# michaelnny/alpha_zero

Measured on AMD Instinct MI355X. Metric: self-play moves/sec (whole node), 9x9 Go @ 200 sims/move, higher is better.
Workload: dtype fp32-class evaluator (f16 hi+lo pairs, 3 MFMA products, fp32 accumulate) / f32-f64 tree

## Files before the change

alpha_zero_amd/csrc/az_conv_sp2p.h:

```cpp
#pragma once
#include "az_conv_sp.h"

#if defined(__HIPCC__)
#define SP2P_NB 12

__device__ __forceinline__ float sp2_fma_f32(float a, float s, float c) {
    float r;
    asm("v_fma_f32 %0, %1, %2, %3" : "=v"(r) : "v"(a), "s"(s), "v"(c));
    return r;
}

struct Sp2pMap {
    unsigned char cell[10 * 16];
};
constexpr Sp2pMap sp2p_map_table = {{
     46,  48,  50,  52,  47,  49,  51,  64,  65,  67,  69,  71,  53,  66,  68,  70,
     10,  12,  14,  16,  11,  13,  15,  28,  29,  31,  33,  35,  17,  30,  32,  34,
     20,  22,  24,  37,  19,  21,  23,  25,  26,  39,  41,  43,  38,  40,  42,  44,
      1,   2,   3,   4,  82,  83,  84,  85,  86,  87,  88,  89,   5,   6,   7,   8,
     55,  56,  57,  58, 136, 137, 138, 139, 140, 141, 142, 143,  59,  60,  61,  62,
     73,  74,  75,  76, 154, 155, 156, 157, 158, 159, 160, 161,  77,  78,  79,  80,
      0,   9,  18,  27,  81,  90,  99, 108, 117, 126, 135, 144,  36,  45,  54,  63,
    127, 129, 131, 133, 128, 130, 132, 145, 146, 148, 150, 152, 134, 147, 149, 151,
     91,  93,  95,  97,  92,  94,  96, 109, 110, 112, 114, 116,  98, 111, 113, 115,
    101, 103, 105, 118, 100, 102, 104, 106, 107, 120, 122, 124, 119, 121, 123, 125,
}};
constexpr int SP2P_NCT = 10, SP2P_KS = 18;
constexpr bool sp2p_tap_off(int pos, int tap) {
    const int yy = pos / SpGeo9::S + tap / 3 - 1, xx = pos % SpGeo9::S + tap % 3 - 1;
    return yy < 0 || yy >= SpGeo9::S || xx < 0 || xx >= SpGeo9::S;
}
constexpr bool sp2p_skip(const Sp2pMap& m, int tile, int tap) {
    for (int n = 0; n < 16; ++n)
        if (!sp2p_tap_off(m.cell[tile * 16 + n] % SpGeo9::P2, tap)) return false;
    return true;
}
constexpr int sp2p_skips(const Sp2pMap& m) {
    int n = 0;
    for (int t = 0; t < SP2P_NCT; ++t)
        for (int tap = 0; tap < 9; ++tap) n += sp2p_skip(m, t, tap) ? 1 : 0;
    return n;
}
constexpr bool sp2p_map_complete(const Sp2pMap& m) {
    bool used[2 * SpGeo9::P2] = {};
    for (int i = 0; i < SP2P_NCT * 16; ++i) {
        const int v = m.cell[i];
        if (v >= 2 * SpGeo9::P2 || v % SpGeo9::P2 == SpGeo9::CORNER || used[v]) return false;
        used[v] = true;
    }
    return true;
}
constexpr bool sp2p_map_conflict_free(const Sp2pMap& m) {
    for (int t = 0; t < SP2P_NCT; ++t) {
        bool bank[16] = {};
        for (int n = 0; n < 16; ++n) {
            const int r = (SpGeo9::cell_of(m.cell[t * 16 + n] % SpGeo9::P2) + ((n >= 4 && n < 12) ? 8 : 0)) & 15;
            if (bank[r]) return false;
            bank[r] = true;
        }
    }
    return true;
}
constexpr bool sp2p_skips_as_designed(const Sp2pMap& m) {
    for (int t = 0; t < SP2P_NCT; ++t)
        for (int tap = 0; tap < 9; ++tap) {
            const bool want = (t == 3 && tap / 3 == 0) || (t == 5 && tap / 3 == 2) || (t == 6 && tap % 3 == 0);
            if (sp2p_skip(m, t, tap) != want) return false;
        }
    return true;
}
constexpr int sp2p_sector_complete(const Sp2pMap& m) {
    int n = 0;
    for (int t = 0; t < SP2P_NCT; ++t)
        for (int a = 0; a < 16; ++a)
            for (int b = 0; b < 16; ++b) {
                const int p = m.cell[t * 16 + a], q = m.cell[t * 16 + b];
                n += (q == p + 1 && p / SpGeo9::P2 == q / SpGeo9::P2) ? 1 : 0;
            }
    return n;
}
static_assert(sp2p_map_complete(sp2p_map_table), "pair map: every position of both boards but the two corners exactly once");
static_assert(sp2p_map_conflict_free(sp2p_map_table), "pair map: conflict-free lane groups in every tile");
static_assert(sp2p_skips_as_designed(sp2p_map_table) && sp2p_skips(sp2p_map_table) == 9, "pair map: the three edge tiles skip 3 taps each, 9 of 90 (tile, tap) pairs");
static_assert(sp2p_sector_complete(sp2p_map_table) == 126, "pair map: 9 rows of both boards in one tile each, 7 whole sectors per row");
static __device__ const Sp2pMap sp2p_map = sp2p_map_table;

constexpr int sp2p_j0(int u) { return u == 0 ? 0 : u == 1 ? 3 : u == 2 ? 5 : 8; }
constexpr int sp2p_nj(int u) { return (u & 1) ? 2 : 3; }
constexpr bool sp2p_has_end(int u) { return u == 0 || u == 3; }
struct Sp2pSched {
    int n;
    int kstart[SP2P_KS + 1];
    int live_n[SP2P_KS];
    unsigned char live[SP2P_KS][3];
    unsigned char t[324], jl[324], tt[324], prod[324], first[324];
};
constexpr Sp2pSched sp2p_sched(int u) {
    Sp2pSched s = {};
    const int j0 = sp2p_j0(u), nj = sp2p_nj(u);
    int first_t[3] = {-1, -1, -1};
    int n = 0;
    for (int t = 0; t < SP2P_KS; ++t) {
        int ln = 0;
        for (int j = 0; j < nj; ++j)
            if (!sp2p_skip(sp2p_map_table, j0 + j, t / 2)) {
                s.live[t][ln++] = (unsigned char)j;
                if (first_t[j] < 0) first_t[j] = t;
            }
        s.live_n[t] = ln;
        s.kstart[t] = n;
        for (int r6 = 0; r6 < 6; ++r6)
            for (int k = 0; k < ln; ++k) {
                const int j = s.live[t][k];
                s.t[n] = (unsigned char)t, s.jl[n] = (unsigned char)j, s.tt[n] = (unsigned char)(r6 / 3), s.prod[n] = (unsigned char)(r6 % 3);
                s.first[n] = first_t[j] == t ? 1 : 0;
                ++n;
            }
    }
    s.kstart[SP2P_KS] = n, s.n = n;
    return s;
}
template <int U> struct Sp2pU {
    static constexpr Sp2pSched S = sp2p_sched(U);
};
static_assert(Sp2pU<0>::S.n + Sp2pU<1>::S.n + Sp2pU<2>::S.n + Sp2pU<3>::S.n == 972, "MFMAs per wave and pair: 1080 less 9 x 12");
static_assert(Sp2pU<1>::S.n == 180, "the top tile shares its unit with the never-skipped tile");

template <bool RES, int U> struct Sp2pK {
    static constexpr int KS = SP2P_KS, S0 = 6, NPIECE = 16;
    static constexpr int E1 = RES ? 4 : 2, PAIR = 2 * E1 + 8, CT_OPS = 2 * PAIR + 2, P2CT = CT_OPS + 1;
    static constexpr int PU = (U + 3) & 3, NU = (U + 1) & 3;
    static constexpr int nj = sp2p_nj(U), j0 = sp2p_j0(U), pnj = sp2p_nj(PU), pj0 = sp2p_j0(PU);
    static constexpr bool END = sp2p_has_end(U), PRE = !sp2p_has_end(PU);
    static constexpr int N = Sp2pU<U>::S.n, KLAST = Sp2pU<U>::S.kstart[KS - 1];
    static constexpr int P1 = 5 * pnj, SBX = S0 + P1 + 1, P2 = pnj * P2CT;
    static constexpr int AVAIL = (END ? KLAST : N - 4) - (SBX + 1);
    typedef SpSpread<P2, SBX + 1, AVAIL> SP;
    static constexpr bool DMA = END;
    static constexpr int PFIRST = SBX + 3, PSTRIDE = U == 0 ? 9 : 6, PLAST = PFIRST + (NPIECE - 1) * PSTRIDE;
    static_assert(SP::MAXPER <= 1, "the previous unit's finishing fits this unit's MFMA gaps");
    static_assert(SBX + 1 < Sp2pU<U>::S.kstart[4] && 2 * nj <= S0, "hand-over early in the unit; residual loads in front of it");
    static_assert(!DMA || (PLAST + 2 * 6 * nj < KLAST && PFIRST > SBX), "pieces behind the barrier that frees the image, well in front of the end barrier");
};
template <bool RES, int U> __host__ __device__ constexpr int sp2p_vm_younger() {
    typedef Sp2pK<RES, U> K;
    int n = 0;
    for (int c = 0; c < K::pnj; ++c)
        for (int st = 0; st < 2; ++st)
            if (K::SP::slot_of(c * K::P2CT + K::P2CT - 2 + st) > K::PLAST) ++n;
    return n;
}

template <bool RES> __global__ void __launch_bounds__(CW_THREADS, 1)
k_conv3x3_sp2p(const unsigned char* __restrict__ x, const _Float16* __restrict__ w, const float* __restrict__ bias,
               const unsigned char* __restrict__ res, unsigned char* __restrict__ y, int npairs, int relu, unsigned* range) {
    typedef SpGeo9 G;
    constexpr int C = 128, CIN = 128, NCH = 16, NCG = 2;
    constexpr int KSUB = 2, KS = SP2P_KS;
    constexpr int NT = 2;
    constexpr int NJ0 = 3, NJ1 = 2, R = 2;
    constexpr int LBLK = G::CELLS * 16, LPLANE = NCH * LBLK, LBUF = 2 * LPLANE;
    constexpr int GBLK = G::P2 * 16, XPLANE = NCH * GBLK, XTILE = 2 * XPLANE;
    constexpr int YPLANE = (C / 8) * GBLK, YTILE = 2 * YPLANE;
    constexpr int NP = (G::CELLS + 63) / 64, SPW = 2 * NCH / 4, NPIECE = NP * SPW;
    constexpr int NF = NT * 2 * KS;
    constexpr int NF_A = 64;
    constexpr int P2CT = Sp2pK<RES, 0>::P2CT, PAIR = Sp2pK<RES, 0>::PAIR, E1 = Sp2pK<RES, 0>::E1, S0 = Sp2pK<RES, 0>::S0;
    static_assert(NPIECE == Sp2pK<RES, 0>::NPIECE && KS % R == 0, "pieces per image; ring phase");
    constexpr int SIDE_BOARD = 8 * NCH * 16 + 16, SIDE0 = 2 * LBUF + 16, XB0 = SIDE0 + SP2P_NB * SIDE_BOARD, XBCT = 4 * 1024;
    __shared__ __attribute__((aligned(1024))) unsigned char lds[XB0 + NJ0 * XBCT];
    static_assert(XB0 + NJ0 * XBCT <= 160 * 1024 && XB0 % 16 == 0, "LDS budget");
    const int tid = threadIdx.x, lane = tid & 63, l15 = lane & 15, kg = lane >> 4;
    const int wave = __builtin_amdgcn_readfirstlane(tid >> 6);
    const int wa = wave >> 1, wb = wave & 1;
    const unsigned lds0 = (unsigned)(size_t)(__attribute__((address_space(3))) unsigned char*)lds;
    int cg, slot, nslot;
    {
        const int b = (int)blockIdx.x, nb = (int)gridDim.x;
        nslot = nb / NCG;
        if (nb % (8 * NCG) == 0) {
            const int xcd = b & 7, k = b >> 3;
            cg = k % NCG;
            slot = xcd + 8 * (k / NCG);
        } else {
            cg = b % NCG;
            slot = b / NCG;
        }
    }
    for (int i = tid; i < (XB0 + NJ0 * XBCT) / 16; i += CW_THREADS) *(cv_u32x4*)(lds + i * 16) = (cv_u32x4){0u, 0u, 0u, 0u};
    CV_BARRIER();
    if (slot >= npairs) return;

    sp_f16x8 wf[NF];
#pragma unroll
    for (int f = 0; f < NF; ++f) {
        const int tt = f / (2 * KS), pl = (f / KS) & 1, st = f % KS;
        wf[f] = *(const sp_f16x8*)(w + ((size_t)((pl * 9 + st / KSUB) * C + cg * 64 + wa * 32 + ((tt + wb) & 1) * 16 + l15)) * CIN + wb * 64 + (st % KSUB) * 32 + kg * 8);
    }
    c6_f32x4 bv;
#pragma unroll
    for (int e = 0; e < 4; ++e) bv[e] = bias[cg * 64 + wa * 32 + wb * 16 + 4 * kg + e];
    const float lo_relu = relu ? 0.0f : -__builtin_inff();
    const float lo_clamp = relu ? 0.0f : -SP_F16_MAX;

    unsigned dsrc[NP];
    unsigned long long dmask[NP];
#pragma unroll
    for (int i = 0; i < NP; ++i) {
        const int p = 64 * i + lane < G::CELLS ? G::pos_of_cell(64 * i + lane) : -1;
        dsrc[i] = (unsigned)((p < 0 ? 0 : p) * 16);
        dmask[i] = __builtin_amdgcn_ballot_w64(p >= 0);
    }
    auto dma_piece = [&](const unsigned char* src, unsigned dstbuf, bool live, int i) {
        const int c = SPW * wave + i / NP, pc = i % NP;
        const unsigned long long base = (unsigned long long)(src + (size_t)c * GBLK);
        const unsigned long long mask = live ? dmask[pc] : 0ull;
        const unsigned dst = dstbuf + (unsigned)(c * LBLK + pc * 1024);
        asm volatile("s_mov_b64 exec, %0\n\ts_mov_b32 m0, %1\n\ts_nop 0\n\tglobal_load_lds_dwordx4 %2, %3 nt\n\ts_mov_b64 exec, -1"
                     :
                     : "s"(mask), "s"(dst), "v"(dsrc[pc]), "s"(base)
                     : "memory");
    };
    unsigned lmap[SP2P_NCT], omap[SP2P_NCT];
#pragma unroll
    for (int j = 0; j < SP2P_NCT; ++j) {
        const int v = sp2p_map.cell[j * 16 + l15], bd = v >= G::P2 ? 1 : 0, pos = v - bd * G::P2;
        lmap[j] = (unsigned)(bd * LBUF + (G::PITCH * (pos / G::S) + pos % G::S) * 16 + kg * LBLK + wb * (8 * LBLK));
        omap[j] = (unsigned)(bd * YTILE + pos * 16 + (kg >> 1) * GBLK + (kg & 1) * 8);
    }
    auto out_off = [&](int j) __attribute__((always_inline)) {
        unsigned v = omap[j];
        asm volatile("" : "+v"(v));
        return v;
    };
    sp_f16x8 bb[R][2][NJ0];
    auto load_frag = [&](int j, int jl, int s, int rs, int pl) __attribute__((always_inline)) {
        const int tap = s / KSUB;
        const int off = ((tap / 3) * G::PITCH + (tap % 3)) * 16 + (s % KSUB) * (4 * LBLK);
        bb[rs][pl][jl] = *(const sp_f16x8*)(lds + lmap[j] + off + pl * LPLANE);
    };
    {
        const unsigned char* src = x + (size_t)slot * (2 * XTILE);
#pragma unroll
        for (int i = 0; i < NPIECE; ++i) dma_piece(src, lds0, true, i);
        asm volatile("s_waitcnt vmcnt(0)" ::: "memory");
        CV_BARRIER();
        static_assert(Sp2pU<0>::S.live_n[0] == NJ0, "the first k-step of a pair has all of U0's tiles");
#pragma unroll
        for (int pl = 0; pl < 2; ++pl)
#pragma unroll
            for (int j = 0; j < NJ0; ++j) load_frag(j, j, 0, 0, pl);
    }
#pragma unroll
    for (int f = 0; f < NF; ++f) {
        if (f < NF_A) asm volatile("" : : "a"(wf[f]));
        else asm volatile("" : : "v"(wf[f]));
    }
    asm volatile("" : : "v"(bv), "v"(lmap[0]), "v"(lmap[SP2P_NCT - 1]), "v"(dsrc[0]), "v"(dsrc[NP - 1]));

    c6_f32x4 accm[2][NJ0][NT], accc[2][NJ0][NT];
    cv_u32x2 rr[2][NJ0][2];
#pragma unroll
    for (int a = 0; a < 2; ++a)
#pragma unroll
        for (int j = 0; j < NJ0; ++j) {
#pragma unroll
            for (int t = 0; t < NT; ++t) accm[a][j][t] = (c6_f32x4){0.0f, 0.0f, 0.0f, 0.0f}, accc[a][j][t] = (c6_f32x4){0.0f, 0.0f, 0.0f, 0.0f};
            rr[a][j][0] = (cv_u32x2){0u, 0u}, rr[a][j][1] = (cv_u32x2){0u, 0u};
        }
    float evv[2] = {0.0f, 0.0f}, sc[2] = {0.0f, 0.0f}, t0 = 0.0f, mx = 0.0f;
    unsigned hpk[2] = {0u, 0u}, lpk[2] = {0u, 0u};
    c6_f32x4 xs = (c6_f32x4){0.0f, 0.0f, 0.0f, 0.0f}, xr = (c6_f32x4){0.0f, 0.0f, 0.0f, 0.0f};
    unsigned char* const xb_mine = lds + XB0 + wave * 1024 + lane * 16;
    const unsigned char* const xb_partner = lds + XB0 + (wave ^ 1) * 1024 + lane * 16;
    auto send_op = [&](int set, int c, int o) {
        if (o < 4) xs[o] = sp2_fma_f32(accc[set][c][1][o], SP_INV_SCALE, accm[set][c][1][o]);
        else *(c6_f32x4*)(xb_mine + c * XBCT) = xs;
    };
    auto fin_op = [&](int set, int c, int mj, unsigned char* out, sp_gptr out_lo, int o, bool store_ok) {
        if (o == 0) {
            xr = *(const c6_f32x4*)(xb_partner + c * XBCT);
            return;
        }
        o -= 1;
        if (o < 2 * PAIR) {
            const int pr = o / PAIR, k = o % PAIR;
            if (k < 2 * E1) {
                const int ei = k / E1, kk = k % E1, e = 2 * pr + ei;
                const unsigned rh = pr == 0 ? rr[set][c][0].x : rr[set][c][0].y, rl = pr == 0 ? rr[set][c][1].x : rr[set][c][1].y;
                if (kk == 0) evv[ei] = fmaf(accc[set][c][0][e], SP_INV_SCALE, accm[set][c][0][e]);
                else if (kk == 1) evv[ei] = cw_add_f32(evv[ei], xr[e]);
                else if (RES && kk == 2) t0 = ei == 0 ? sp_mix_join<0>(rh, rl) : sp_mix_join<1>(rh, rl);
                else if (RES && kk == 3) evv[ei] = cw_add_f32(evv[ei], t0);
            } else {
                const int kk = k - 2 * E1;
                if (kk == 0) mx = sp_max3_abs(mx, evv[0], evv[1]);
                else if (kk == 1) evv[0] = __builtin_amdgcn_fmed3f(evv[0], lo_clamp, SP_F16_MAX);
                else if (kk == 2) evv[1] = __builtin_amdgcn_fmed3f(evv[1], lo_clamp, SP_F16_MAX);
                else if (kk == 3) hpk[pr] = sp_cvt_pk(evv[0], evv[1]);
                else if (kk == 4) sc[0] = sp_mix_diff<0>(hpk[pr], evv[0]);
                else if (kk == 5) sc[1] = sp_mix_diff<1>(hpk[pr], evv[1]);
                else if (kk == 6) lpk[pr] = sp_scale_cvt_lo(sc[0]);
                else lpk[pr] = sp_scale_cvt_hi(lpk[pr], sc[1]);
            }
        } else {
            const unsigned gq = out_off(mj);
            if (o == 2 * PAIR) {
                if (store_ok) *(cv_u32x2*)(out + gq) = (cv_u32x2){hpk[0], hpk[1]};
            } else if (store_ok) *(__attribute__((address_space(1))) cv_u32x2*)(out_lo + gq) = (cv_u32x2){lpk[0], lpk[1]};
        }
    };

    const bool copier = tid < 8 * NCH;
    int csrc, cdst;
    {
        constexpr int KF = NCH / 4;
        const int c = copier ? tid : 0, ks = c % KF, pl = (c / KF) & 1, tp = (c / (2 * KF)) & 3, g4 = c / (8 * KF);
        csrc = (pl * NCH + 4 * ks + g4) * LBLK + (G::CELL0 + G::PITCH * (G::S - 2 + (tp >> 1)) + (tp & 1)) * 16;
        cdst = SIDE0 + c * 16;
    }
    cv_u32x4 ctmp = (cv_u32x4){0u, 0u, 0u, 0u};

    int it = 0, cb = 0;
    unsigned char* yprev = y;
    sp_gptr yprev_lo = (sp_gptr)(unsigned long long)y;
    for (int pair = slot; pair < npairs; pair += nslot, ++it) {
        const bool has_next = pair + nslot < npairs;
        const unsigned char* bsrc = x + (size_t)pair * (2 * XTILE) + XTILE;
        const unsigned char* nsrc = x + (size_t)(has_next ? pair + nslot : pair) * (2 * XTILE);
        const size_t yo = (size_t)pair * (2 * YTILE) + (size_t)(cg * 8 + wa * 4 + wb * 2) * GBLK;
        const unsigned char* rbase = RES ? res + yo : nullptr;
        unsigned char* ybase = y + yo;
        unsigned long long rlo = (unsigned long long)(RES ? res + yo : y + yo) + YPLANE, ylo = (unsigned long long)(y + yo) + YPLANE;
        asm volatile("" : "+s"(rlo), "+s"(ylo));
        const sp_gcptr rbase_lo = (sp_gcptr)rlo;
        const sp_gptr ybase_lo = (sp_gptr)ylo;
        const bool have_prev = it > 0;
        auto unit = [&](auto UC) __attribute__((always_inline)) {
            constexpr int u = decltype(UC)::value, set = u & 1, pset = set ^ 1;
            typedef Sp2pK<RES, u> K;
            typedef typename K::SP SP;
            constexpr int nj = K::nj, j0 = K::j0, pj0 = K::pj0, nj0 = sp2p_j0(K::NU);
            unsigned char* pout = u == 0 ? yprev : ybase;
            const sp_gptr pout_lo = u == 0 ? yprev_lo : ybase_lo;
            const bool pstore = u > 0 || have_prev;
            cp_for_each([&](auto SC) __attribute__((always_inline)) {
                constexpr int sl = decltype(SC)::value;
                constexpr int t = Sp2pU<u>::S.t[sl], jl = Sp2pU<u>::S.jl[sl], tt = Sp2pU<u>::S.tt[sl], prod = Sp2pU<u>::S.prod[sl];
                constexpr int qi = sl - Sp2pU<u>::S.kstart[t];
                constexpr bool first = Sp2pU<u>::S.first[sl] != 0;
                if constexpr (K::END && sl == K::KLAST) {
                    constexpr int VM_YOUNGER = sp2p_vm_younger<RES, u>();
                    static_assert(VM_YOUNGER < 63, "vmcnt field");
                    if (pstore) asm volatile("s_waitcnt vmcnt(%0)" ::"n"(VM_YOUNGER) : "memory");
                    else asm volatile("s_waitcnt vmcnt(0)" ::: "memory");
                    CV_BARRIER();
                }
                if constexpr (K::PRE && sl == S0 - 1) CV_BARRIER();
                if constexpr (sl == K::SBX) CV_BARRIER();
                constexpr int fa = (tt * 2 + (prod == 2 ? 1 : 0)) * KS + t, pl = prod == 1 ? 1 : 0;
                static_assert(!first || fa < NF_A, "an accumulator's first MFMA reads its weights from the AGPRs");
                if constexpr (prod == 0) {
                    if constexpr (first && tt == 0) sp_mfma_ac(accm[set][jl][tt], wf[fa], bb[t % R][pl][jl], bv);
                    else if constexpr (first) sp_mfma_a0(accm[set][jl][tt], wf[fa], bb[t % R][pl][jl]);
                    else if constexpr (fa < NF_A) sp_mfma_a(accm[set][jl][tt], wf[fa], bb[t % R][pl][jl]);
                    else sp_mfma_v(accm[set][jl][tt], wf[fa], bb[t % R][pl][jl]);
                } else if constexpr (prod == 1) {
                    if constexpr (first) sp_mfma_a0(accc[set][jl][tt], wf[fa], bb[t % R][pl][jl]);
                    else if constexpr (fa < NF_A) sp_mfma_a(accc[set][jl][tt], wf[fa], bb[t % R][pl][jl]);
                    else sp_mfma_v(accc[set][jl][tt], wf[fa], bb[t % R][pl][jl]);
                } else {
                    if constexpr (fa < NF_A) sp_mfma_a(accc[set][jl][tt], wf[fa], bb[t % R][pl][jl]);
                    else sp_mfma_v(accc[set][jl][tt], wf[fa], bb[t % R][pl][jl]);
                }
                {
                    constexpr bool lsame = t + 1 < KS;
                    constexpr int lu = lsame ? u : K::NU, lt = lsame ? t + 1 : 0, lj0 = lsame ? j0 : nj0;
                    constexpr int lnj = Sp2pU<lu>::S.live_n[lt];
                    static_assert(2 * lnj <= 6 * Sp2pU<u>::S.live_n[t], "a fragment per MFMA gap");
                    if constexpr (qi < 2 * lnj) {
                        constexpr int ljl = Sp2pU<lu>::S.live[lt][qi % lnj];
                        load_frag(lj0 + ljl, ljl, lt, (t + 1) % R, qi / lnj);
                    }
                }
                if constexpr (sl >= S0 && sl < S0 + K::P1) send_op(pset, (sl - S0) / 5, (sl - S0) % 5);
                if constexpr (sl > K::SBX) {
                    constexpr int o = SP::cum(sl - 1);
                    if constexpr (o < SP::cum(sl)) fin_op(pset, o / P2CT, pj0 + o / P2CT, pout, pout_lo, o % P2CT, pstore);
                }
                if constexpr (RES && sl < 2 * nj) {
                    constexpr int rj = sl >> 1, rp = sl & 1;
                    if constexpr (rp == 0) rr[set][rj][rp] = *(const cv_u32x2*)(rbase + out_off(j0 + rj));
                    else rr[set][rj][rp] = *(const __attribute__((address_space(1))) cv_u32x2*)(rbase_lo + out_off(j0 + rj));
                }
                __builtin_amdgcn_sched_barrier(0);
                if constexpr (K::DMA && sl >= K::PFIRST && sl <= K::PLAST && (sl - K::PFIRST) % K::PSTRIDE == 0) {
                    if constexpr (u == 0) dma_piece(bsrc, lds0 + LBUF, true, (sl - K::PFIRST) / K::PSTRIDE);
                    else dma_piece(nsrc, lds0, has_next, (sl - K::PFIRST) / K::PSTRIDE);
                    __builtin_amdgcn_sched_barrier(0);
                }
                if constexpr ((u == 0 || u == 2) && sl == Sp2pU<u>::S.kstart[3] - 1) {
                    if (copier) ctmp = *(const cv_u32x4*)(lds + csrc + (u == 2 ? LBUF : 0));
                    __builtin_amdgcn_sched_barrier(0);
                }
                if constexpr ((u == 0 || u == 2) && sl == Sp2pU<u>::S.kstart[6] - 1) {
                    if (copier) *(cv_u32x4*)(lds + cdst + (cb + (u == 2 ? 1 : 0)) * SIDE_BOARD) = ctmp;
                    __builtin_amdgcn_sched_barrier(0);
                }
            }, typename CpMakeSeq<K::N>::type{});
        };
        unit(CpInt<0>{});
        unit(CpInt<1>{});
        unit(CpInt<2>{});
        unit(CpInt<3>{});
        yprev = ybase, yprev_lo = ybase_lo;
        cb += 2;
        if (cb == SP2P_NB || !has_next) {
            const int n_ok = cb, it0 = it - (cb / 2 - 1);
            c6_f32x4 cm[NT], cc[NT];
            constexpr int KF = NCH / 4;
            const unsigned char* sb = lds + SIDE0 + l15 * SIDE_BOARD + kg * (8 * KF * 16);
            const int nb = l15 < n_ok ? l15 : 0;
            const size_t board = 2 * ((size_t)slot + (size_t)(it0 + (nb >> 1)) * nslot) + (nb & 1);
            const size_t co = board * YTILE + (size_t)(cg * 8 + wa * 4 + wb * 2 + (kg >> 1)) * GBLK + G::CORNER * 16 + (kg & 1) * 8;
            if (RES) {
                rr[0][0][0] = *(const cv_u32x2*)(res + co);
                rr[0][0][1] = *(const cv_u32x2*)(res + co + YPLANE);
            }
            cp_for_each([&](auto TC) __attribute__((always_inline)) {
                constexpr int u = decltype(TC)::value, tp = u / KSUB, ks = u % KSUB;
                constexpr int fw = ((tp >> 1) * 3 + 1 + (tp & 1)) * KSUB + ks;
                const sp_f16x8 bh = *(const sp_f16x8*)(sb + ((tp * 2 + 0) * KF + wb * KSUB + ks) * 16);
                const sp_f16x8 bl = *(const sp_f16x8*)(sb + ((tp * 2 + 1) * KF + wb * KSUB + ks) * 16);
#pragma unroll
                for (int tt = 0; tt < NT; ++tt) {
                    const int fh = (tt * 2 + 0) * KS + fw, fl = (tt * 2 + 1) * KS + fw;
                    if (u == 0 && tt == 0) sp_mfma_ac(cm[tt], wf[fh], bh, bv);
                    else if (u == 0) sp_mfma_a0(cm[tt], wf[fh], bh);
                    else if (fh < NF_A) sp_mfma_a(cm[tt], wf[fh], bh);
                    else sp_mfma_v(cm[tt], wf[fh], bh);
                    if (u == 0) sp_mfma_a0(cc[tt], wf[fh], bl);
                    else if (fh < NF_A) sp_mfma_a(cc[tt], wf[fh], bl);
                    else sp_mfma_v(cc[tt], wf[fh], bl);
                    if (fl < NF_A) sp_mfma_a(cc[tt], wf[fl], bh);
                    else sp_mfma_v(cc[tt], wf[fl], bh);
                }
                __builtin_amdgcn_sched_barrier(0);
            }, typename CpMakeSeq<4 * KSUB>::type{});
            asm volatile("s_nop 15\n\ts_nop 15" : "+v"(cm[0]), "+v"(cc[0]), "+v"(cm[1]), "+v"(cc[1]));
            c6_f32x4 hs;
#pragma unroll
            for (int e = 0; e < 4; ++e) hs[e] = fmaf(cc[1][e], SP_INV_SCALE, cm[1][e]);
            *(c6_f32x4*)(xb_mine) = hs;
            CV_BARRIER();
            const c6_f32x4 hr = *(const c6_f32x4*)(xb_partner);
            float v[4];
#pragma unroll
            for (int e = 0; e < 4; ++e) v[e] = fmaf(cc[0][e], SP_INV_SCALE, cm[0][e]) + hr[e];
            if (RES) {
                const cv_u32x2 rh = rr[0][0][0], rl = rr[0][0][1];
                v[0] += sp_join(sp_lo16(rh.x), sp_lo16(rl.x));
                v[1] += sp_join(sp_hi16(rh.x), sp_hi16(rl.x));
                v[2] += sp_join(sp_lo16(rh.y), sp_lo16(rl.y));
                v[3] += sp_join(sp_hi16(rh.y), sp_hi16(rl.y));
            }
            _Float16 h[4], l[4];
#pragma unroll
            for (int e = 0; e < 4; ++e) {
                if (l15 < n_ok) mx = fmaxf(mx, fabsf(v[e]));
                v[e] = fmaxf(v[e], lo_relu);
                sp_split(v[e], h[e], l[e]);
            }
            if (l15 < n_ok) {
                *(cv_u32x2*)(y + co) = (cv_u32x2){sp_pack(h[0], h[1]), sp_pack(h[2], h[3])};
                *(cv_u32x2*)(y + co + YPLANE) = (cv_u32x2){sp_pack(l[0], l[1]), sp_pack(l[2], l[3])};
            }
            cb = 0;
            CV_BARRIER();
        }
    }
    asm volatile("s_nop 15\n\ts_nop 15" : "+v"(accm[1][0][0]), "+v"(accm[1][1][0]), "+v"(accc[1][0][0]), "+v"(accc[1][1][0]), "+v"(accm[1][0][1]), "+v"(accm[1][1][1]),
                 "+v"(accc[1][0][1]), "+v"(accc[1][1][1]));
#pragma unroll
    for (int c = 0; c < NJ1; ++c)
#pragma unroll
        for (int o = 0; o < 5; ++o) send_op(1, c, o);
    CV_BARRIER();
#pragma unroll
    for (int c = 0; c < NJ1; ++c)
#pragma unroll
        for (int o = 0; o < P2CT; ++o) fin_op(1, c, sp2p_j0(3) + c, yprev, yprev_lo, o, true);
    sp_range_report(mx, range);
}
#endif
```

Before: 7274.

## Share LDS input fragments across row-shifted tiles in the interior conv units

Reorders the pair map so that the tiles within units 0 and 3 are vertical row shifts of one another. Those units then run a skewed schedule over row steps, in which one LDS fragment read feeds every live tile. The goal is fewer LDS fragment reads per wave (about 252 instead of 324), so less LDS bandwidth and issue pressure in the MFMA conv loop. In exchange the step count and MFMA ordering change, and so do the barrier and DMA slot positions that are tied to kstart. That may perturb the hand-tuned overlap of finishing work and prefetch.

```diff
diff --git a/alpha_zero_amd/csrc/az_conv_sp2p.h b/alpha_zero_amd/csrc/az_conv_sp2p.h
--- a/alpha_zero_amd/csrc/az_conv_sp2p.h
+++ b/alpha_zero_amd/csrc/az_conv_sp2p.h
@@ -14,16 +14,16 @@
     unsigned char cell[10 * 16];
 };
 constexpr Sp2pMap sp2p_map_table = {{
-     46,  48,  50,  52,  47,  49,  51,  64,  65,  67,  69,  71,  53,  66,  68,  70,
-     10,  12,  14,  16,  11,  13,  15,  28,  29,  31,  33,  35,  17,  30,  32,  34,
-     20,  22,  24,  37,  19,  21,  23,  25,  26,  39,  41,  43,  38,  40,  42,  44,
+     16,  17,  48,  49,  10,  11,  12,  13,  14,  15,  46,  47,  50,  51,  52,  53,
+     25,  26,  57,  58,  19,  20,  21,  22,  23,  24,  55,  56,  59,  60,  61,  62,
+     34,  35,  66,  67,  28,  29,  30,  31,  32,  33,  64,  65,  68,  69,  70,  71,
       1,   2,   3,   4,  82,  83,  84,  85,  86,  87,  88,  89,   5,   6,   7,   8,
-     55,  56,  57,  58, 136, 137, 138, 139, 140, 141, 142, 143,  59,  60,  61,  62,
+    118, 119, 120, 121,  37,  38,  39,  40,  41,  42,  43,  44, 122, 123, 124, 125,
      73,  74,  75,  76, 154, 155, 156, 157, 158, 159, 160, 161,  77,  78,  79,  80,
       0,   9,  18,  27,  81,  90,  99, 108, 117, 126, 135, 144,  36,  45,  54,  63,
-    127, 129, 131, 133, 128, 130, 132, 145, 146, 148, 150, 152, 134, 147, 149, 151,
-     91,  93,  95,  97,  92,  94,  96, 109, 110, 112, 114, 116,  98, 111, 113, 115,
-    101, 103, 105, 118, 100, 102, 104, 106, 107, 120, 122, 124, 119, 121, 123, 125,
+     97,  98, 129, 130,  91,  92,  93,  94,  95,  96, 127, 128, 131, 132, 133, 134,
+    106, 107, 138, 139, 100, 101, 102, 103, 104, 105, 136, 137, 140, 141, 142, 143,
+    115, 116, 147, 148, 109, 110, 111, 112, 113, 114, 145, 146, 149, 150, 151, 152,
 }};
 constexpr int SP2P_NCT = 10, SP2P_KS = 18;
 constexpr bool sp2p_tap_off(int pos, int tap) {
@@ -88,51 +88,97 @@
 constexpr int sp2p_j0(int u) { return u == 0 ? 0 : u == 1 ? 3 : u == 2 ? 5 : 8; }
 constexpr int sp2p_nj(int u) { return (u & 1) ? 2 : 3; }
 constexpr bool sp2p_has_end(int u) { return u == 0 || u == 3; }
+constexpr bool sp2p_row_shifts(const Sp2pMap& m, int u) {
+    const int j0 = sp2p_j0(u), nj = sp2p_nj(u);
+    for (int j = 0; j < nj; ++j) {
+        for (int n = 0; n < 16; ++n)
+            if (m.cell[(j0 + j) * 16 + n] != m.cell[j0 * 16 + n] + j * SpGeo9::S) return false;
+        for (int tap = 0; tap < 9; ++tap)
+            if (sp2p_skip(m, j0 + j, tap)) return false;
+    }
+    return true;
+}
+static_assert(sp2p_row_shifts(sp2p_map_table, 0) && sp2p_row_shifts(sp2p_map_table, 3), "pair map: the local tiles of a board are row shifts of one another");
+static_assert(!sp2p_row_shifts(sp2p_map_table, 1) && !sp2p_row_shifts(sp2p_map_table, 2), "pair map: the units with edge tiles read a fragment per tile");
+constexpr int SP2P_MAXST = 6 * 5;
 struct Sp2pSched {
-    int n;
-    int kstart[SP2P_KS + 1];
-    int live_n[SP2P_KS];
-    unsigned char live[SP2P_KS][3];
-    unsigned char t[324], jl[324], tt[324], prod[324], first[324];
+    int n, ns;
+    bool shared;
+    int kstart[SP2P_MAXST + 1];
+    int live_n[SP2P_MAXST];
+    unsigned char live[SP2P_MAXST][3];
+    unsigned char frow[SP2P_MAXST], fcol[SP2P_MAXST], fkh[SP2P_MAXST];
+    unsigned char st[324], jl[324], wk[324], tt[324], prod[324], first[324];
+    constexpr int nfrag(int step) const { return shared ? 1 : live_n[step]; }
+    constexpr int reads() const {
+        int r = 0;
+        for (int i = 0; i < ns; ++i) r += 2 * nfrag(i);
+        return r;
+    }
 };
 constexpr Sp2pSched sp2p_sched(int u) {
     Sp2pSched s = {};
     const int j0 = sp2p_j0(u), nj = sp2p_nj(u);
-    int first_t[3] = {-1, -1, -1};
+    s.shared = sp2p_row_shifts(sp2p_map_table, u);
+    s.ns = s.shared ? 6 * (nj + 2) : SP2P_KS;
+    int first_st[3] = {-1, -1, -1};
     int n = 0;
-    for (int t = 0; t < SP2P_KS; ++t) {
-        int ln = 0;
-        for (int j = 0; j < nj; ++j)
-            if (!sp2p_skip(sp2p_map_table, j0 + j, t / 2)) {
-                s.live[t][ln++] = (unsigned char)j;
-                if (first_t[j] < 0) first_t[j] = t;
-            }
-        s.live_n[t] = ln;
-        s.kstart[t] = n;
+    for (int i = 0; i < s.ns; ++i) {
+        const int row = i / 6, col = (i / 2) % 3, kh = i % 2;
+        int ln = 0, wk[3] = {};
+        for (int j = 0; j < nj; ++j) {
+            const int dy1 = s.shared ? row - j : row;
+            if (dy1 < 0 || dy1 > 2 || sp2p_skip(sp2p_map_table, j0 + j, dy1 * 3 + col)) continue;
+            wk[ln] = (dy1 * 3 + col) * 2 + kh;
+            s.live[i][ln++] = (unsigned char)j;
+            if (first_st[j] < 0) first_st[j] = i;
+        }
+        s.live_n[i] = ln;
+        s.kstart[i] = n;
+        s.frow[i] = (unsigned char)row, s.fcol[i] = (unsigned char)col, s.fkh[i] = (unsigned char)kh;
         for (int r6 = 0; r6 < 6; ++r6)
             for (int k = 0; k < ln; ++k) {
-                const int j = s.live[t][k];
-                s.t[n] = (unsigned char)t, s.jl[n] = (unsigned char)j, s.tt[n] = (unsigned char)(r6 / 3), s.prod[n] = (unsigned char)(r6 % 3);
-                s.first[n] = first_t[j] == t ? 1 : 0;
+                const int j = s.live[i][k];
+                s.st[n] = (unsigned char)i, s.jl[n] = (unsigned char)j, s.wk[n] = (unsigned char)wk[k], s.tt[n] = (unsigned char)(r6 / 3), s.prod[n] = (unsigned char)(r6 % 3);
+                s.first[n] = first_st[j] == i ? 1 : 0;
                 ++n;
             }
     }
-    s.kstart[SP2P_KS] = n, s.n = n;
+    s.kstart[s.ns] = n, s.n = n;
     return s;
+}
+constexpr bool sp2p_chains_ascend(const Sp2pSched& s, int u) {
+    for (int j = 0; j < sp2p_nj(u); ++j)
+        for (int r6 = 0; r6 < 6; ++r6) {
+            int next = 0;
+            for (int sl = 0; sl < s.n; ++sl) {
+                if (s.jl[sl] != j || s.tt[sl] * 3 + s.prod[sl] != r6) continue;
+                while (next < SP2P_KS && sp2p_skip(sp2p_map_table, sp2p_j0(u) + j, next / 2)) ++next;
+                if (s.wk[sl] != next++) return false;
+            }
+            while (next < SP2P_KS && sp2p_skip(sp2p_map_table, sp2p_j0(u) + j, next / 2)) ++next;
+            if (next != SP2P_KS) return false;
+        }
+    return true;
 }
 template <int U> struct Sp2pU {
     static constexpr Sp2pSched S = sp2p_sched(U);
+    static_assert(sp2p_chains_ascend(S, U), "an accumulator's chain: its live weight k-steps, each once, ascending");
+    static_assert(S.ns % 2 == 0, "the fragment ring (2 slots) is in the same phase at every unit's first step");
 };
 static_assert(Sp2pU<0>::S.n + Sp2pU<1>::S.n + Sp2pU<2>::S.n + Sp2pU<3>::S.n == 972, "MFMAs per wave and pair: 1080 less 9 x 12");
 static_assert(Sp2pU<1>::S.n == 180, "the top tile shares its unit with the never-skipped tile");
+static_assert(Sp2pU<0>::S.ns == 30 && Sp2pU<3>::S.ns == 24 && Sp2pU<0>::S.n == 324 && Sp2pU<3>::S.n == 216, "the skewed units: 1, 2, 3, 2, 1 and 1, 2, 2, 1 live tiles per row set");
+static_assert(Sp2pU<0>::S.reads() == 60 && Sp2pU<1>::S.reads() == 60 && Sp2pU<2>::S.reads() == 84 && Sp2pU<3>::S.reads() == 48,
+              "fragment reads per wave and pair: 252 (324 with a fragment per tile in every unit)");
 
 template <bool RES, int U> struct Sp2pK {
-    static constexpr int KS = SP2P_KS, S0 = 6, NPIECE = 16;
+    static constexpr int NS = Sp2pU<U>::S.ns, S0 = 6, NPIECE = 16;
     static constexpr int E1 = RES ? 4 : 2, PAIR = 2 * E1 + 8, CT_OPS = 2 * PAIR + 2, P2CT = CT_OPS + 1;
     static constexpr int PU = (U + 3) & 3, NU = (U + 1) & 3;
     static constexpr int nj = sp2p_nj(U), j0 = sp2p_j0(U), pnj = sp2p_nj(PU), pj0 = sp2p_j0(PU);
     static constexpr bool END = sp2p_has_end(U), PRE = !sp2p_has_end(PU);
-    static constexpr int N = Sp2pU<U>::S.n, KLAST = Sp2pU<U>::S.kstart[KS - 1];
+    static constexpr int N = Sp2pU<U>::S.n, KLAST = Sp2pU<U>::S.kstart[NS - 1];
     static constexpr int P1 = 5 * pnj, SBX = S0 + P1 + 1, P2 = pnj * P2CT;
     static constexpr int AVAIL = (END ? KLAST : N - 4) - (SBX + 1);
     typedef SpSpread<P2, SBX + 1, AVAIL> SP;
@@ -234,10 +280,13 @@
         return v;
     };
     sp_f16x8 bb[R][2][NJ0];
-    auto load_frag = [&](int j, int jl, int s, int rs, int pl) __attribute__((always_inline)) {
-        const int tap = s / KSUB;
-        const int off = ((tap / 3) * G::PITCH + (tap % 3)) * 16 + (s % KSUB) * (4 * LBLK);
-        bb[rs][pl][jl] = *(const sp_f16x8*)(lds + lmap[j] + off + pl * LPLANE);
+    auto frag_req = [&](auto LU, auto LT, auto QC) __attribute__((always_inline)) {
+        constexpr int lu = decltype(LU)::value, lt = decltype(LT)::value, q = decltype(QC)::value;
+        constexpr int nf = Sp2pU<lu>::S.nfrag(lt), pl = q / nf;
+        constexpr int jr = Sp2pU<lu>::S.shared ? 0 : Sp2pU<lu>::S.live[lt][q % nf];
+        constexpr int off = (Sp2pU<lu>::S.frow[lt] * G::PITCH + Sp2pU<lu>::S.fcol[lt]) * 16 + Sp2pU<lu>::S.fkh[lt] * (4 * LBLK);
+        static_assert(pl < 2, "two planes per fragment");
+        bb[lt % R][pl][jr] = *(const sp_f16x8*)(lds + lmap[sp2p_j0(lu) + jr] + off + pl * LPLANE);
     };
     {
         const unsigned char* src = x + (size_t)slot * (2 * XTILE);
@@ -245,11 +294,9 @@
         for (int i = 0; i < NPIECE; ++i) dma_piece(src, lds0, true, i);
         asm volatile("s_waitcnt vmcnt(0)" ::: "memory");
         CV_BARRIER();
-        static_assert(Sp2pU<0>::S.live_n[0] == NJ0, "the first k-step of a pair has all of U0's tiles");
-#pragma unroll
-        for (int pl = 0; pl < 2; ++pl)
-#pragma unroll
-            for (int j = 0; j < NJ0; ++j) load_frag(j, j, 0, 0, pl);
+        static_assert(Sp2pU<0>::S.nfrag(0) == 1, "the first step of a pair reads one fragment");
+        frag_req(CpInt<0>{}, CpInt<0>{}, CpInt<0>{});
+        frag_req(CpInt<0>{}, CpInt<0>{}, CpInt<1>{});
     }
 #pragma unroll
     for (int f = 0; f < NF; ++f) {
@@ -340,13 +387,14 @@
             constexpr int u = decltype(UC)::value, set = u & 1, pset = set ^ 1;
             typedef Sp2pK<RES, u> K;
             typedef typename K::SP SP;
-            constexpr int nj = K::nj, j0 = K::j0, pj0 = K::pj0, nj0 = sp2p_j0(K::NU);
+            constexpr int nj = K::nj, j0 = K::j0, pj0 = K::pj0;
             unsigned char* pout = u == 0 ? yprev : ybase;
             const sp_gptr pout_lo = u == 0 ? yprev_lo : ybase_lo;
             const bool pstore = u > 0 || have_prev;
             cp_for_each([&](auto SC) __attribute__((always_inline)) {
                 constexpr int sl = decltype(SC)::value;
-                constexpr int t = Sp2pU<u>::S.t[sl], jl = Sp2pU<u>::S.jl[sl], tt = Sp2pU<u>::S.tt[sl], prod = Sp2pU<u>::S.prod[sl];
+                constexpr int t = Sp2pU<u>::S.st[sl], jl = Sp2pU<u>::S.jl[sl], wk = Sp2pU<u>::S.wk[sl], tt = Sp2pU<u>::S.tt[sl], prod = Sp2pU<u>::S.prod[sl];
+                constexpr int jb = Sp2pU<u>::S.shared ? 0 : jl;
                 constexpr int qi = sl - Sp2pU<u>::S.kstart[t];
                 constexpr bool first = Sp2pU<u>::S.first[sl] != 0;
                 if constexpr (K::END && sl == K::KLAST) {
@@ -358,30 +406,27 @@
                 }
                 if constexpr (K::PRE && sl == S0 - 1) CV_BARRIER();
                 if constexpr (sl == K::SBX) CV_BARRIER();
-                constexpr int fa = (tt * 2 + (prod == 2 ? 1 : 0)) * KS + t, pl = prod == 1 ? 1 : 0;
+                constexpr int fa = (tt * 2 + (prod == 2 ? 1 : 0)) * KS + wk, pl = prod == 1 ? 1 : 0;
                 static_assert(!first || fa < NF_A, "an accumulator's first MFMA reads its weights from the AGPRs");
                 if constexpr (prod == 0) {
-                    if constexpr (first && tt == 0) sp_mfma_ac(accm[set][jl][tt], wf[fa], bb[t % R][pl][jl], bv);
-                    else if constexpr (first) sp_mfma_a0(accm[set][jl][tt], wf[fa], bb[t % R][pl][jl]);
-                    else if constexpr (fa < NF_A) sp_mfma_a(accm[set][jl][tt], wf[fa], bb[t % R][pl][jl]);
-                    else sp_mfma_v(accm[set][jl][tt], wf[fa], bb[t % R][pl][jl]);
+                    if constexpr (first && tt == 0) sp_mfma_ac(accm[set][jl][tt], wf[fa], bb[t % R][pl][jb], bv);
+                    else if constexpr (first) sp_mfma_a0(accm[set][jl][tt], wf[fa], bb[t % R][pl][jb]);
+                    else if constexpr (fa < NF_A) sp_mfma_a(accm[set][jl][tt], wf[fa], bb[t % R][pl][jb]);
+                    else sp_mfma_v(accm[set][jl][tt], wf[fa], bb[t % R][pl][jb]);
                 } else if constexpr (prod == 1) {
-                    if constexpr (first) sp_mfma_a0(accc[set][jl][tt], wf[fa], bb[t % R][pl][jl]);
-                    else if constexpr (fa < NF_A) sp_mfma_a(accc[set][jl][tt], wf[fa], bb[t % R][pl][jl]);
-                    else sp_mfma_v(accc[set][jl][tt], wf[fa], bb[t % R][pl][jl]);
+                    if constexpr (first) sp_mfma_a0(accc[set][jl][tt], wf[fa], bb[t % R][pl][jb]);
+                    else if constexpr (fa < NF_A) sp_mfma_a(accc[set][jl][tt], wf[fa], bb[t % R][pl][jb]);
+                    else sp_mfma_v(accc[set][jl][tt], wf[fa], bb[t % R][pl][jb]);
                 } else {
-                    if constexpr (fa < NF_A) sp_mfma_a(accc[set][jl][tt], wf[fa], bb[t % R][pl][jl]);
-                    else sp_mfma_v(accc[set][jl][tt], wf[fa], bb[t % R][pl][jl]);
+                    if constexpr (fa < NF_A) sp_mfma_a(accc[set][jl][tt], wf[fa], bb[t % R][pl][jb]);
+                    else sp_mfma_v(accc[set][jl][tt], wf[fa], bb[t % R][pl][jb]);
                 }
                 {
-                    constexpr bool lsame = t + 1 < KS;
-                    constexpr int lu = lsame ? u : K::NU, lt = lsame ? t + 1 : 0, lj0 = lsame ? j0 : nj0;
-                    constexpr int lnj = Sp2pU<lu>::S.live_n[lt];
-                    static_assert(2 * lnj <= 6 * Sp2pU<u>::S.live_n[t], "a fragment per MFMA gap");
-                    if constexpr (qi < 2 * lnj) {
-                        constexpr int ljl = Sp2pU<lu>::S.live[lt][qi % lnj];
-                        load_frag(lj0 + ljl, ljl, lt, (t + 1) % R, qi / lnj);
-                    }
+                    constexpr bool lsame = t + 1 < K::NS;
+                    constexpr int lu = lsame ? u : K::NU, lt = lsame ? t + 1 : 0;
+                    constexpr int nreq = 2 * Sp2pU<lu>::S.nfrag(lt);
+                    static_assert(nreq <= 6 * Sp2pU<u>::S.live_n[t], "a fragment per MFMA gap");
+                    if constexpr (qi < nreq) frag_req(CpInt<lu>{}, CpInt<lt>{}, CpInt<qi>{});
                 }
                 if constexpr (sl >= S0 && sl < S0 + K::P1) send_op(pset, (sl - S0) / 5, (sl - S0) % 5);
                 if constexpr (sl > K::SBX) {
```

New measurement: 7381 (median of 6 runs). 1.01x the previous value.
